# 0411tony/Yue

Hardware: AMD Instinct MI355X
Metric: BPR triplet-updates/sec at k=128 (S-round semantics, user rows sequential; the reference's exact sequential semantics: secondary.exact) (higher is better)
Workload: dtype f32

## Files before the change

### yue_amd/csrc/bpr_host.hip

```cpp
#include "host_common.hpp"

#include "train_kernels.hpp"
#include "round_kernels.hpp"

using yue_host::fail;
using yue_host::kr_of;
static_assert(yue::kNllSlots == yue_host::kNllSlotsHost && yue::kHeaderSlack == yue_host::kHeaderSlackHost, "host_common.hpp mirrors these");

namespace {

yue::TrainArgs make_args(yue_ctx *c, double lr, double regU, double regI) {
    yue::TrainArgs a{};
    a.P = c->P.p; a.Q = c->Q.p; a.dP = c->dP.p; a.dQ = c->dQ.p;
    a.stage = c->Q.p ? c->Q.p + (size_t)c->n * c->k : nullptr;
    a.ev_u = c->ev_u.p; a.ev_i = c->ev_i.p; a.ev_j = c->ev_j.p;
    a.indptr = c->indptr.p; a.indices = c->indices.p;
    a.nll_slots = c->scal.p;
    a.m = c->m; a.n = c->n; a.k = c->k;
    a.lr = lr;
    a.ru = (float)(lr * regU);
    a.ri = (float)(lr * regI);
    a.neg_lo = 0; a.neg_range = (int32_t)c->n;
    return a;
}

void launch_level(yue_ctx *c, const yue::TrainArgs &a, int64_t e0, int64_t e1) {
    const int tpw = (int)std::min<int64_t>(64, std::max<int64_t>(1, (e1 - e0) / 4096));
    const int64_t waves = (e1 - e0 + tpw - 1) / tpw;
    const dim3 grid((unsigned)((waves + 3) / 4)), block(256);
    switch (kr_of(c->k)) {
        case 1: hipLaunchKernelGGL(yue::k_bpr_level<1>, grid, block, 0, c->stream, a, e0, e1, tpw); break;
        case 2: hipLaunchKernelGGL(yue::k_bpr_level<2>, grid, block, 0, c->stream, a, e0, e1, tpw); break;
        default: hipLaunchKernelGGL(yue::k_bpr_level<4>, grid, block, 0, c->stream, a, e0, e1, tpw); break;
    }
}

int tpw_of(const yue_ctx *c, bool meta) {
    if (c->opt_round_tpw) return c->opt_round_tpw;
    const int kr = kr_of(c->k);
    return kr == 4 ? 4 : kr == 2 ? 8 : meta ? 8 : 16;
}

constexpr int64_t kMetaRangeMax = 37 * 1024;
constexpr int64_t kMetaRangesMax = 12;
constexpr int64_t kRoundGenerationsMax = 6;
constexpr double kRoundEventsPerItemRow = 4.0;
// ... 174 lines not shown
            default: return fail(YUE_ERR_ARG, "item matrices of 2 GiB and more: only the default events-per-wave setting (round_tpw = 0)");
        }
    } else
#define YUE_RM(KR_, TPW_) hipLaunchKernelGGL((yue::k_round_m<KR_, TPW_>), grid, block, 0, c->stream, a, ra, a.ev_u, a.ev_i, a.ev_j, mi, mj); break;
    switch (kr_of(c->k) * 16 + tpw) {
        case 1 * 16 + 8: YUE_RM(1, 8)
        case 1 * 16 + 16: YUE_RM(1, 16)
        case 2 * 16 + 8: YUE_RM(2, 8)
        case 4 * 16 + 4: YUE_RM(4, 4)
        case 1 * 16 + 4: YUE_RM(1, 4)
        case 2 * 16 + 4: YUE_RM(2, 4)
        case 1 * 16 + 2: YUE_RM(1, 2)
        case 2 * 16 + 2: YUE_RM(2, 2)
        default: return fail(YUE_ERR_ARG, "unsupported (k, TPW) combination");
    }
#undef YUE_RM
    launch_round_fold(c, a, e0, e1, round_index);
    return YUE_OK;
}

int launch_round_u(yue_ctx *c, const yue::TrainArgs &a, int64_t u0, int64_t u1, int64_t e0, int64_t e1, int64_t round_index) {
    yue::RoundUArgs ra{};
    ra.u_begin = u0; ra.u_end = u1; ra.ev_ptr = c->d_ev_ptr.p; ra.e_begin = e0; ra.e_end = e1; ra.staged = c->staged ? 1 : 0; ra.margins = c->margins.p;
    ra.psq_slots = c->psq_in_rounds ? c->psq_slots.p : nullptr;
    const int64_t blocks = (u1 - u0 + 3) / 4;
    if (blocks == 0) return YUE_OK;
    const dim3 grid((unsigned)blocks), block(256);
    const uint32_t *mi = c->meta_i.p, *mj = c->meta_j.p;
#define YUE_RU(KR_) do { if (c->opt_round_fast) hipLaunchKernelGGL((yue::k_round_u<KR_, true>), grid, block, 0, c->stream, a, ra, a.ev_i, a.ev_j, mi, mj); \
                         else hipLaunchKernelGGL((yue::k_round_u<KR_, false>), grid, block, 0, c->stream, a, ra, a.ev_i, a.ev_j, mi, mj); } while (0)
    switch (kr_of(c->k)) {
        case 1: YUE_RU(1); break;
        case 2: YUE_RU(2); break;
        default: YUE_RU(4); break;
    }
#undef YUE_RU
    launch_round_fold(c, a, e0, e1, round_index);
    return YUE_OK;
}

template <typename F>
int run_rounds(yue_ctx *c, yue::TrainArgs a, const std::vector<int64_t> &bounds, int apply_p, F after_round, bool meta = false, const std::vector<int64_t> *user_blocks = nullptr) {
    const int64_t R = (int64_t)bounds.size() - 1;
    int64_t widest = 0;
    for (int64_t r = 0; r < R; ++r) widest = std::max(widest, bounds[(size_t)r + 1] - bounds[(size_t)r]);
    if (widest >= (1ll << 24)) meta = false;
    const bool fits31 = (c->n + 2 * widest) * (int64_t)c->k * 4 < (1ll << 31);
// ... 57 lines not shown
        c->ev_triplets[c->ev_used] = bounds.back() - bounds.front();
        c->ev_launches[c->ev_used] = (int64_t)ne.size();
        c->ev_used++;
    }
    return YUE_OK;
}

void reset_round_state(yue_ctx *c) {
    (void)hipStreamSynchronize(c->stream);
    if (c->cnt0.p) (void)hipMemsetAsync(c->cnt0.p, 0, c->cnt0.n * sizeof(unsigned long long), c->stream);
    if (c->cnt1.p) (void)hipMemsetAsync(c->cnt1.p, 0, c->cnt1.n * sizeof(unsigned long long), c->stream);
    if (c->cntp0.p) (void)hipMemsetAsync(c->cntp0.p, 0, c->cntp0.n * sizeof(uint32_t), c->stream);
    if (c->cntp1.p) (void)hipMemsetAsync(c->cntp1.p, 0, c->cntp1.n * sizeof(uint32_t), c->stream);
    if (c->dP.p) (void)hipMemsetAsync(c->dP.p, 0, c->dP.n * sizeof(float), c->stream);
    if (c->dQ.p) (void)hipMemsetAsync(c->dQ.p, 0, c->dQ.n * sizeof(float), c->stream);
    (void)hipStreamSynchronize(c->stream);
}


}

namespace yue_host {
int zero_scalars(yue_ctx *c) {
    HIPCHK(hipMemsetAsync(c->scal.p, 0, (yue::kNllSlots + 8) * sizeof(double), c->stream));
    return YUE_OK;
}

int read_scalars(yue_ctx *c, double *nll, double *sp, double *sq) {
    double *sc = c->scal.p + yue::kNllSlots;
    hipLaunchKernelGGL(yue::k_sum_slots, dim3(1), dim3(64), 0, c->stream, c->scal.p, yue::kNllSlots, sc);
    double h[3];
    HIPCHK(hipMemcpyAsync(h, sc, sizeof h, hipMemcpyDeviceToHost, c->stream));
    HIPCHK(hipStreamSynchronize(c->stream));
    if (nll) *nll = h[0];
    if (sp) *sp = h[1];
    if (sq) *sq = h[2];
    return YUE_OK;
}

int sumsq_async(yue_ctx *c, const double *p_slots) {
    double *sc = c->scal.p + yue::kNllSlots;
    HIPCHK(hipMemsetAsync(sc + 1, 0, 2 * sizeof(double), c->stream));
    if (p_slots) hipLaunchKernelGGL(yue::k_sum_slots, dim3(1), dim3(64), 0, c->stream, p_slots, yue::kNllSlots, sc + 1);
    else hipLaunchKernelGGL(yue::k_sumsq, dim3(2048), dim3(256), 0, c->stream, c->P.p, c->m * c->k, sc + 1);
    hipLaunchKernelGGL(yue::k_sumsq, dim3(2048), dim3(256), 0, c->stream, c->Q.p, c->n * c->k, sc + 2);
    return YUE_OK;
}

int upload_triplets(yue_ctx *c, const int32_t *u, const int32_t *i, const int32_t *j, int64_t T, bool validate) {
    for (int64_t t = 0; validate && t < T; ++t) {
        if (u[t] < 0 || u[t] >= c->m || i[t] < 0 || i[t] >= c->n || j[t] >= c->n)
            return fail(YUE_ERR_ARG, "triplet " + std::to_string(t) + " out of range");
    }
// ... 143 lines not shown
    a.U = c->P.p; a.V = c->Q.p; a.gU = c->dP.p; a.gV = c->dQ.p; a.k = c->k; a.u = c->xu.p; a.i = c->xi.p; a.j = c->xj.p; a.T = T;
    a.reg = (float)reg; a.loss_slots = c->scal.p;
    const dim3 grid((unsigned)(((T + 31) / 32 + 3) / 4));
    switch (kr_of(c->k)) {
        case 1: hipLaunchKernelGGL(yue::k_mb_grad<1>, grid, dim3(256), 0, c->stream, a); break;
        case 2: hipLaunchKernelGGL(yue::k_mb_grad<2>, grid, dim3(256), 0, c->stream, a); break;
        default: hipLaunchKernelGGL(yue::k_mb_grad<4>, grid, dim3(256), 0, c->stream, a); break;
    }
    const double b1 = 0.9, b2 = 0.999;
    const float lr_t = (float)(lr * std::sqrt(1.0 - std::pow(b2, (double)step)) / (1.0 - std::pow(b1, (double)step)));
    const int64_t mk = c->m * (int64_t)c->k, nk = c->n * (int64_t)c->k;
    hipLaunchKernelGGL(yue::k_adam, dim3((unsigned)std::min<int64_t>(8192, (mk + 255) / 256)), dim3(256), 0, c->stream, c->P.p, c->aU_m.p, c->aU_v.p, c->dP.p, mk, lr_t, 0.9f, 0.999f, 1e-8f);
    hipLaunchKernelGGL(yue::k_adam, dim3((unsigned)std::min<int64_t>(8192, (nk + 255) / 256)), dim3(256), 0, c->stream, c->Q.p, c->aV_m.p, c->aV_v.p, c->dQ.p, nk, lr_t, 0.9f, 0.999f, 1e-8f);
    HIPCHK(hipGetLastError());
    return read_scalars(c, loss_out, nullptr, nullptr);
}

int yue_sample_negatives(yue_ctx *c, uint64_t seed, uint32_t epoch, int32_t *j_out) {
    if (!c || !c->have_inter || !j_out) return fail(YUE_ERR_ARG, "yue_sample_negatives: no interactions uploaded");
    HIPCHK(hipSetDevice(c->device));
    yue::TrainArgs a = make_args(c, 0, 0, 0);
    a.seed = seed; a.epoch = epoch;
    if (c->E > 0) {
        hipLaunchKernelGGL(yue::k_sample, dim3((unsigned)((c->E + 255) / 256)), dim3(256), 0, c->stream, a, c->E);
        HIPCHK(hipGetLastError());
        HIPCHK(hipMemcpyAsync(j_out, c->ev_j.p, c->E * sizeof(int32_t), hipMemcpyDeviceToHost, c->stream));
    }
    HIPCHK(hipStreamSynchronize(c->stream));
    return YUE_OK;
}

int yue_sumsq(yue_ctx *c, double *sp, double *sq) {
    if (!c || !c->have_factors) return fail(YUE_ERR_ARG, "yue_sumsq: no factors uploaded");
    HIPCHK(hipSetDevice(c->device));
    int rc = sumsq_async(c);
    if (rc) return rc;
    double h[2];
    HIPCHK(hipMemcpyAsync(h, c->scal.p + yue::kNllSlots + 1, sizeof h, hipMemcpyDeviceToHost, c->stream));
    HIPCHK(hipStreamSynchronize(c->stream));
    if (sp) *sp = h[0];
    if (sq) *sq = h[1];
    return YUE_OK;
}

int yue_bpr_epoch(yue_ctx *c, uint64_t seed, uint32_t epoch, int64_t round_events, double lr, double regU, double regI,
                  double *nll_out, double *sumsqP_out, double *sumsqQ_out) {
    if (!c || !c->have_factors || !c->have_inter) return fail(YUE_ERR_ARG, "yue_bpr_epoch: upload factors and interactions first");
    if (round_events < 0) return fail(YUE_ERR_ARG, "yue_bpr_epoch: round_events must be positive (or 0 for the device's default)");
    HIPCHK(hipSetDevice(c->device));
    yue::TrainArgs a = make_args(c, lr, regU, regI);
    a.seed = seed + 0x632BE59BD9B4E019ull * (uint64_t)c->rank;
    a.epoch = epoch;
    int rc = zero_scalars(c);
    if (rc) return rc;
    const int64_t E = c->E;
    if (E > 0) hipLaunchKernelGGL(yue::k_sample, dim3((unsigned)((E + 255) / 256)), dim3(256), 0, c->stream, a, E);
    if (c->opt_epoch_exact) {
        if (yue_host::on_communicator(c) && c->nranks > 1) return fail(YUE_ERR_ARG, "yue_bpr_epoch: option epoch_exact runs on one GPU (the sequential order spans all item shards)");
        if ((rc = yue_host::chain_epoch(c, lr, regU, regI))) return rc;
        if ((rc = sumsq_async(c))) return rc;
        return read_scalars(c, nll_out, sumsqP_out, sumsqQ_out);
    }
    std::vector<int64_t> bounds;
    double tot[2] = {(double)E, (double)c->n};
    if (yue_host::on_communicator(c)) {
        if ((rc = yue_allreduce_f64(c, tot, 2))) return rc;
        if ((rc = zero_scalars(c))) return rc;
    }
    const double etot = tot[0];
    if (round_events == 0 && (rc = default_round_events(c, tot[1] / c->nranks, &round_events))) return rc;
    int64_t ub = 1, group = 1;
    if ((rc = yue_epoch_plan(c->m, c->k, round_events, etot, c->nranks, &ub, &group, nullptr))) return rc;
    if (!yue_host::on_communicator(c)) group = std::max<int64_t>(1, (c->m + ub - 1) / ub);
    else group = std::max<int64_t>(1, ((int64_t)c->opt_comm_group_mb << 20) / std::max<int64_t>(1, ub * c->k * 4));
    std::vector<int64_t> ublock;
    for (int64_t u0 = 0; u0 < c->m; u0 += ub) { ublock.push_back(u0); bounds.push_back(c->h_ev_ptr[(size_t)u0]); }
    ublock.push_back(c->m); bounds.push_back(E);
    const int64_t R = (int64_t)ublock.size() - 1;
    const bool seq_user = !yue_host::on_communicator(c) && c->opt_round_user_seq && meta_path_fits(c);
    if (seq_user) {
        HIPCHK(c->d_ev_ptr.resize((size_t)c->m + 1));
        if (!c->d_ev_ptr_valid) {
            HIPCHK(hipMemcpyAsync(c->d_ev_ptr.p, c->h_ev_ptr.data(), ((size_t)c->m + 1) * sizeof(int64_t), hipMemcpyHostToDevice, c->stream));
            c->d_ev_ptr_valid = true;
        }
        HIPCHK(c->margins.resize((size_t)std::max<int64_t>(E, 1)));
    }
    c->psq_in_rounds = seq_user && c->all_users_have_events && E > 0;
    if (c->psq_in_rounds) {
        HIPCHK(c->psq_slots.resize((size_t)yue::kNllSlots));
        HIPCHK(hipMemsetAsync(c->psq_slots.p, 0, (size_t)yue::kNllSlots * sizeof(double), c->stream));
    }
    c->last_round_user_seq = 0;
    auto after = [&](int64_t r) -> int {
        if (seq_user && !c->bigq) { c->last_round_user_seq = 1; return YUE_OK; }
        if ((r + 1) % group != 0 && r + 1 != R) return YUE_OK;
        const int64_t g_first = ublock[(size_t)(r - (r % group))], g_last = ublock[(size_t)r + 1];
        const int64_t first = g_first * c->k, count = (g_last - g_first) * c->k;
        const dim3 grid((unsigned)std::min<int64_t>(4096, (count + 255) / 256));
        if (!yue_host::on_communicator(c)) {
            hipLaunchKernelGGL(yue::k_apply_range, grid, dim3(256), 0, c->stream, c->P.p, c->dP.p, first, count);
            return YUE_OK;
        }
        HIPCHK(hipEventRecord(c->ev_rounds, c->stream));
        HIPCHK(hipStreamWaitEvent(c->comm_stream, c->ev_rounds, 0));
        c->comm_collectives += 1;
        c->comm_bytes += (double)count * sizeof(float);
        if (const int rcr = yue_host::reduce_user_block(c, first, count, c->comm_stream)) return rcr;
        hipLaunchKernelGGL(yue::k_apply_range, grid, dim3(256), 0, c->comm_stream, c->P.p, c->dP.p, first, count);
        return YUE_OK;
    };
    c->comm_collectives = 0; c->comm_bytes = 0.0; c->comm_wait_ms = 0.0;
    if ((rc = run_rounds(c, a, bounds, 0, after, meta_path_fits(c), seq_user ? &ublock : nullptr))) { reset_round_state(c); return rc; }
    if (c->last_round_user_seq && E > 0)
        hipLaunchKernelGGL(yue::k_loss_margins, dim3(2048), dim3(256), 0, c->stream, c->margins.p, c->ev_j.p, E, c->scal.p);
    const bool psq_done = c->psq_in_rounds && c->last_round_user_seq;
    c->psq_in_rounds = false;
    if (yue_host::on_communicator(c)) {
        HIPCHK(hipEventRecord(c->ev_t_rounds, c->stream));
        HIPCHK(hipEventRecord(c->ev_t_comm, c->comm_stream));
    }
    HIPCHK(hipEventRecord(c->ev_comm, c->comm_stream));
    HIPCHK(hipStreamWaitEvent(c->stream, c->ev_comm, 0));
    c->comm_compute_waits = 1;
    HIPCHK(hipGetLastError());
    if ((rc = sumsq_async(c, psq_done ? c->psq_slots.p : nullptr))) return rc;
    if ((rc = read_scalars(c, nll_out, sumsqP_out, sumsqQ_out))) return rc;
    if (yue_host::on_communicator(c)) {
        float ms = 0.f;
        HIPCHK(hipEventSynchronize(c->ev_t_comm));
        HIPCHK(hipEventElapsedTime(&ms, c->ev_t_rounds, c->ev_t_comm));
        c->comm_wait_ms = ms > 0.f ? ms : 0.0;
    }
    return YUE_OK;
}

int yue_epoch_plan(int64_t m, int k, int64_t round_events, double events_total, int nranks,
                   int64_t *user_block, int64_t *blocks_per_group, int64_t *n_blocks) {
    if (m <= 0 || k <= 0 || round_events <= 0 || nranks < 1 || !(events_total >= 0.0)) return fail(YUE_ERR_ARG, "yue_epoch_plan: bad argument");
    const double per_user = events_total / (double)nranks / (double)m;
    const int64_t ub = std::max<int64_t>(1, (int64_t)std::floor((double)round_events / std::max(per_user, 1e-9) + 0.5));
    if (user_block) *user_block = ub;
    if (blocks_per_group) *blocks_per_group = std::max<int64_t>(1, (8ll << 20) / std::max<int64_t>(1, ub * k * 4));
    if (n_blocks) *n_blocks = (m + ub - 1) / ub;
    return YUE_OK;
}

int yue_default_round_events(yue_ctx *c, int64_t *out) {
    if (!c || !c->have_factors || !out) return fail(YUE_ERR_ARG, "yue_default_round_events: upload factors first (the value depends on k)");
    HIPCHK(hipSetDevice(c->device));
// ... 56 lines not shown
    else if (key == "scan_batch") *value = c->opt_scan_batch;
    else if (key == "scan_two_phase") *value = c->opt_scan_two_phase;
    else if (key == "fism_lds") *value = c->opt_fism_lds;
    else if (key == "fism_inplace") *value = c->opt_fism_inplace;
    else if (key == "scan_growth") *value = c->opt_scan_growth;
    else if (key == "scan_filter_ub") *value = c->opt_scan_filter_ub;
    else if (key == "scan_streams") *value = c->opt_scan_streams;
    else if (key == "scan_slabs") *value = c->opt_scan_slabs;
    else if (key == "scan_streams_min_users") *value = c->opt_scan_streams_min_users;
    else if (key == "scan_last_chunks") *value = c->scan_chunks;
    else if (key == "scan_last_few_users") *value = c->scan_few_users;
    else if (key == "scan_last_settle") *value = c->scan_settle;
    else if (key == "topn_true") *value = c->opt_topn_true;
    else if (key == "round_stage") *value = c->opt_round_stage;
    else if (key == "round_last_stage_max") *value = c->last_stage_max;
    else if (key == "round_meta") *value = c->opt_round_meta;
    else if (key == "comm_group_mb") *value = c->opt_comm_group_mb;
    else if (key == "round_cus_reserved") *value = c->opt_round_cus_reserved;
    else if (key == "comm_last_compute_waits") *value = c->comm_compute_waits;
    else if (key == "round_user_seq") *value = c->opt_round_user_seq;
    else if (key == "round_fast") *value = c->opt_round_fast;
    else if (key == "round_last_user_seq") *value = c->last_round_user_seq;
    else if (key == "round_bucket") *value = c->opt_round_bucket;
    else if (key == "fold_blocks") *value = c->opt_fold_blocks;
    else if (key == "round_tpw") *value = c->opt_round_tpw;
    else if (key == "epoch_exact") *value = c->opt_epoch_exact;
    else if (key == "replay_levels") *value = c->opt_replay_levels;
    else if (key == "chain_waves") *value = c->opt_chain_waves;
    else if (key == "chain_split") *value = c->opt_chain_split;
    else if (key == "chain_fast") *value = c->opt_chain_fast;
    else if (key == "chain_xcd") *value = c->opt_chain_xcd;
    else if (key == "chain_last_us") *value = c->chain_kernel_us;
    else if (key == "chain_ring") *value = c->opt_chain_ring;
    else if (key == "chain_spin") *value = c->opt_chain_spin;
    else if (key == "chain_last_runs") *value = c->chain_runs;
    else if (key == "chain_last_waves") *value = c->chain_waves;
    else if (key == "replay_last_levels") *value = c->replay_levels;
    else if (key == "round_path") *value = fold_path(c) ? 1 : 0;
    else if (key.compare(0, 5, "wrmf_") == 0) return yue_host::wrmf_get_option(c, key, value);
    else if (key.compare(0, 4, "knn_") == 0) return yue_host::knn_get_option(c, key, value);
    else if (key.compare(0, 4, "ipf_") == 0) return yue_host::ipf_get_option(c, key, value);
    else return fail(YUE_ERR_ARG, "yue_get_option: unknown option " + key);
    return YUE_OK;
}

int yue_set_option(yue_ctx *c, const char *name, int64_t value) {
// ... 25 lines not shown
        hipStream_t fresh = nullptr;
        if (value == 0) HIPCHK(hipStreamCreateWithFlags(&fresh, hipStreamNonBlocking));
        else {
            std::vector<uint32_t> mask((size_t)(cus + 31) / 32, 0u);
            for (int cu = 0; cu < cus - (int)value; ++cu) mask[(size_t)cu / 32] |= 1u << (cu % 32);
            HIPCHK(hipExtStreamCreateWithCUMask(&fresh, (uint32_t)mask.size(), mask.data()));
        }
        (void)hipStreamDestroy(c->stream);
        c->stream = fresh;
        c->opt_round_cus_reserved = (int)value;
        return YUE_OK;
    }
    if (key == "round_user_seq") { c->opt_round_user_seq = value != 0; return YUE_OK; }
    if (key == "round_fast") { c->opt_round_fast = value != 0; return YUE_OK; }
    if (key == "epoch_exact") { c->opt_epoch_exact = value != 0; return YUE_OK; }
    if (key == "replay_levels") { c->opt_replay_levels = value != 0; return YUE_OK; }
    if (key == "chain_split") { if (value < -1 || value > 1) return fail(YUE_ERR_ARG, "yue_set_option: chain_split must be -1, 0 or 1"); c->opt_chain_split = (int)value; return YUE_OK; }
    if (key == "chain_fast") { c->opt_chain_fast = value != 0; return YUE_OK; }
    if (key == "chain_xcd") { c->opt_chain_xcd = value != 0; return YUE_OK; }
    if (key == "chain_ring") { if (value != 0 && value != 8 && value != 16) return fail(YUE_ERR_ARG, "yue_set_option: chain_ring must be 0, 8 or 16"); c->opt_chain_ring = (int)value; return YUE_OK; }
    if (key == "chain_waves") { if (value < 0 || value > 8) return fail(YUE_ERR_ARG, "yue_set_option: chain_waves must be 0..8"); c->opt_chain_waves = (int)value; return YUE_OK; }
    if (key == "chain_spin") { if (value < 0 || value > 0x7fffffff) return fail(YUE_ERR_ARG, "yue_set_option: chain_spin out of range"); c->opt_chain_spin = value; return YUE_OK; }
    if (key == "round_bucket") { c->opt_round_bucket = value != 0; return YUE_OK; }
    if (key == "fold_blocks") { if (value < 1 || value > 65536) return fail(YUE_ERR_ARG, "yue_set_option: fold_blocks out of range"); c->opt_fold_blocks = (int)value; return YUE_OK; }
#ifdef YUE_STAMPS
    if (key == "debug_stamp_launch") { c->stamp_launch = value; c->update_launches = 0; return YUE_OK; }
#endif
    if (key == "round_tpw") {
        if (value != 0 && value != 2 && value != 4 && value != 8 && value != 16) return fail(YUE_ERR_ARG, "yue_set_option: round_tpw must be 0, 2, 4, 8 or 16");
        if (value == 8 && kr_of(c->k) == 4) return fail(YUE_ERR_ARG, "yue_set_option: round_tpw 8 needs k <= 128");
        if (value == 16 && kr_of(c->k) != 1) return fail(YUE_ERR_ARG, "yue_set_option: round_tpw 16 needs k <= 64");
        c->opt_round_tpw = (int)value;
        return YUE_OK;
    }
    if (key.compare(0, 5, "wrmf_") == 0) return yue_host::wrmf_set_option(c, key, value);
    if (key.compare(0, 4, "knn_") == 0) return yue_host::knn_set_option(c, key, value);
    if (key.compare(0, 4, "ipf_") == 0) return yue_host::ipf_set_option(c, key, value);
    return fail(YUE_ERR_ARG, "yue_set_option: unknown option " + key);
}

#ifdef YUE_STAMPS
int yue_debug_get_stamps(yue_ctx *c, unsigned long long *out, int64_t max_waves, int64_t *n_waves) {
    HIPCHK(hipStreamSynchronize(c->stream));
    const int64_t w = std::min(max_waves, c->stamp_waves);
    if (w > 0) HIPCHK(hipMemcpy(out, c->stamps.p, (size_t)w * 64, hipMemcpyDeviceToHost));
    *n_waves = w;
// ... 6 lines not shown
```

### yue_amd/csrc/core_host.hip

```cpp
#include "host_common.hpp"

namespace yue_host {
thread_local std::string g_err;
int fail(int code, const std::string &msg) { g_err = msg; return code; }
}
using yue_host::fail;
void yue_comm_release(yue_ctx *c);

extern "C" {

const char *yue_last_error(void) { return yue_host::g_err.c_str(); }
int yue_version(void) { return 1; }

int yue_ctx_create(int device, yue_ctx **out) {
    if (!out) return fail(YUE_ERR_ARG, "yue_ctx_create: out is NULL");
    int ndev = 0;
    HIPCHK(hipGetDeviceCount(&ndev));
    if (ndev <= 0) return fail(YUE_ERR_HIP, "no HIP device visible: libyue_hip needs an MI355X (no CPU fallback exists)");
    if (device < 0 || device >= ndev) return fail(YUE_ERR_ARG, "device ordinal out of range");
    HIPCHK(hipSetDevice(device));
    yue_ctx *c = new yue_ctx();
    c->device = device;
    const auto init = [c]() -> int {
        HIPCHK(hipStreamCreateWithFlags(&c->stream, hipStreamNonBlocking));
        HIPCHK(hipStreamCreateWithFlags(&c->comm_stream, hipStreamNonBlocking));
        HIPCHK(hipEventCreateWithFlags(&c->ev_rounds, hipEventDisableTiming));
        HIPCHK(hipEventCreateWithFlags(&c->ev_comm, hipEventDisableTiming));
        HIPCHK(hipEventCreate(&c->ev_t_rounds));
        HIPCHK(hipEventCreate(&c->ev_t_comm));
        HIPCHK(hipEventCreate(&c->ev_scan0));
        HIPCHK(hipEventCreate(&c->ev_scan1));
        HIPCHK(c->scal.resize(yue_host::kNllSlotsHost + 8));
        return YUE_OK;
    };
    const int rc = init();
    if (rc) { const std::string msg = yue_host::g_err; (void)yue_ctx_destroy(c); yue_host::g_err = msg; return rc; }
    *out = c;
    return YUE_OK;
}

int yue_ctx_destroy(yue_ctx *c) {
    if (!c) return YUE_OK;
    (void)hipSetDevice(c->device);
    if (c->stream) (void)hipStreamSynchronize(c->stream);
    if (c->comm_stream) (void)hipStreamSynchronize(c->comm_stream);
    yue_comm_release(c);
    if (c->comm_stream) (void)hipStreamDestroy(c->comm_stream);
    if (c->ev_rounds) (void)hipEventDestroy(c->ev_rounds);
    if (c->ev_comm) (void)hipEventDestroy(c->ev_comm);
    if (c->ev_t_rounds) (void)hipEventDestroy(c->ev_t_rounds);
    if (c->ev_t_comm) (void)hipEventDestroy(c->ev_t_comm);
    if (c->ev_scan0) (void)hipEventDestroy(c->ev_scan0);
    if (c->ev_chain0) (void)hipEventDestroy(c->ev_chain0);
    if (c->ev_chain1) (void)hipEventDestroy(c->ev_chain1);
    if (c->ev_scan1) (void)hipEventDestroy(c->ev_scan1);
// ... 110 lines not shown
```

### yue_amd/csrc/host_common.hpp

```cpp
#pragma once
#include "../../include/yue_hip.h"

#include <hip/hip_runtime.h>

#include <algorithm>
#include <cmath>
#include <cstdio>
#include <cstdlib>
#include <cstring>
#include <string>
#include <vector>

struct ncclComm;
struct yue_wrmf;
struct yue_knn;
struct yue_ipf;

namespace yue_host {

int fail(int code, const std::string &msg);

#define HIPCHK(expr)                                                                              \
    do {                                                                                          \
        hipError_t e_ = (expr);                                                                   \
        if (e_ != hipSuccess)                                                                     \
            return yue_host::fail(YUE_ERR_HIP, std::string(#expr) + ": " + hipGetErrorString(e_)); \
    } while (0)

template <typename T>
struct DevBuf {
    T *p = nullptr;
    size_t n = 0;
    hipError_t resize(size_t count) {
        if (count <= n && p) return hipSuccess;
        if (p) { hipError_t e = hipFree(p); p = nullptr; n = 0; if (e != hipSuccess) return e; }
        if (count == 0) return hipSuccess;
        hipError_t e = hipMalloc((void **)&p, count * sizeof(T));
        if (e == hipSuccess) n = count;
        return e;
    }
    void release() { if (p) (void)hipFree(p); p = nullptr; n = 0; }
};

constexpr int kNllSlotsHost = 1024;
constexpr int kHeaderSlackHost = 16;

inline int kr_of(int k) { return k <= 64 ? 1 : k <= 128 ? 2 : 4; }

}

using yue_host::DevBuf;

struct yue_ctx {
    int device = 0;
    hipStream_t stream = nullptr;
    int64_t m = 0, n = 0, E = 0, nnz = 0;
    int k = 0;
    bool have_factors = false, have_inter = false;
    DevBuf<float> P, Q, dP, dQ;
    DevBuf<float> margins;
    DevBuf<double> psq_slots;
    DevBuf<unsigned long long> cnt0, cnt1;
    DevBuf<uint32_t> cntp0, cntp1;
    DevBuf<uint32_t> tab0, tab1;
    bool staged = false;
    bool bigq = false;
    DevBuf<uint32_t> meta_i, meta_j;
    DevBuf<unsigned long long> round_rows;
    DevBuf<uint2> fold, bk_touch;
    DevBuf<uint32_t> bk_ptr;
    DevBuf<int64_t> d_bounds;
    std::vector<int64_t> h_bounds;
#ifdef YUE_STAMPS
    DevBuf<unsigned long long> stamps;
    int64_t stamp_launch = -1, update_launches = 0, stamp_waves = 0;
#endif
    DevBuf<int32_t> ev_u, ev_i, ev_j, indices;
    DevBuf<int64_t> indptr;
    DevBuf<int32_t> xu, xi, xj, xk;
    DevBuf<double> x_loss;
    DevBuf<float> aU_m, aU_v, aV_m, aV_v;
    int64_t adam_m = 0, adam_n = 0; int adam_k = 0;
    DevBuf<double> scal;
    std::vector<int64_t> h_ev_ptr;
// ... 6 lines not shown
    DevBuf<int64_t> s_mask_ptr;
    DevBuf<float> s_scores, s_row, s_norms;
    double scan_ms = 0.0;
    int64_t scan_events = 0, scan_rescored = 0, scan_tiles_done = 0, scan_tiles_total = 0;
    DevBuf<unsigned long long> s_work;
    DevBuf<unsigned short> s_qb;
    DevBuf<uint32_t> s_masks;
    int opt_scan_two_phase = 1;
    int64_t opt_scan_streams_min_users = 262144;
    int opt_scan_slabs = 4;
    int opt_scan_streams = 2;
    int opt_scan_filter_ub = 3;
    int opt_scan_growth = 0;
    int scan_chunks = 0;
    int scan_used_bf16 = 0;
    int opt_scan_f32 = 0;
    int opt_scan_batch = 0;
    int opt_round_tpw = 0;
    int opt_topn_true = 0;
    int scan_settle = 0;
    int last_stage_max = 0;
    int opt_round_stage = 1;
    int opt_round_bucket = 0;
    int opt_fold_blocks = 1536;
    int opt_round_user_seq = 1;
    int opt_round_fast = 1;
    int last_round_user_seq = 0;
    int opt_comm_group_mb = 8;
    int opt_round_cus_reserved = 0;
    int64_t comm_compute_waits = 0;
    int opt_round_meta = 1;
    int timing_stride = 0;
    std::vector<std::pair<hipEvent_t, hipEvent_t>> ev_pool;
    std::vector<int64_t> ev_triplets, ev_launches;
    size_t ev_used = 0;
    DevBuf<double> fP, fBi, f_coef, f_x, f_hist, f_scores, f_out_sc;
    DevBuf<float> fQ;
    DevBuf<int64_t> f_ptr;
    DevBuf<int32_t> f_items, f_negs, f_ids, f_flags;
    DevBuf<int64_t> f_uq_ptr, f_neg_ptr;
    DevBuf<int32_t> f_uq_items, f_loc_i, f_loc_j;
    DevBuf<float> f_wq, f_dQ;
    DevBuf<double> f_wp, f_wb, f_dP, f_dB;
    DevBuf<unsigned> f_cnt;
    int64_t fn = 0;
    int fk = 0;
// ... 17 lines not shown
    int64_t opt_chain_spin = 0;
    int64_t chain_runs = 0, chain_waves = 0, chain_groups = 0, chain_kernel_us = 0, replay_levels = 0;
    hipEvent_t ev_chain0 = nullptr, ev_chain1 = nullptr;
    ncclComm *comm = nullptr;
    int rank = 0, nranks = 1;
    hipStream_t comm_stream = nullptr;
    hipEvent_t ev_rounds = nullptr, ev_comm = nullptr;
    hipEvent_t ev_t_rounds = nullptr, ev_t_comm = nullptr;
    int (*seam_reduce)(void *host, int64_t count, int dtype, void *user) = nullptr;
    void *seam_user = nullptr;
    std::vector<float> seam_buf;
    int64_t comm_collectives = 0;
    double comm_bytes = 0.0, comm_wait_ms = 0.0;
    int comm_version = 0, comm_nranks_reported = 0;
    hipEvent_t ev_scan0 = nullptr, ev_scan1 = nullptr;
    yue_wrmf *wrmf = nullptr;
    yue_knn *knn = nullptr;
    yue_ipf *ipf = nullptr;
};

namespace yue_host {
inline bool on_communicator(const yue_ctx *c) { return c->comm != nullptr || c->seam_reduce != nullptr; }
int zero_scalars(yue_ctx *c);
int read_scalars(yue_ctx *c, double *nll, double *sp, double *sq);
int sumsq_async(yue_ctx *c, const double *p_slots = nullptr);
int upload_triplets(yue_ctx *c, const int32_t *u, const int32_t *i, const int32_t *j, int64_t T, bool validate);
int reduce_user_block(yue_ctx *c, int64_t first, int64_t count, hipStream_t stream);
int chain_epoch(yue_ctx *c, double lr, double regU, double regI);
int chain_stream(yue_ctx *c, int64_t T, double lr, double regU, double regI);
void wrmf_release(yue_ctx *c);
int wrmf_set_option(yue_ctx *c, const std::string &key, int64_t value);
int wrmf_get_option(yue_ctx *c, const std::string &key, int64_t *value);
void knn_release(yue_ctx *c);
int knn_set_option(yue_ctx *c, const std::string &key, int64_t value);
int knn_get_option(yue_ctx *c, const std::string &key, int64_t *value);
void ipf_release(yue_ctx *c);
int ipf_set_option(yue_ctx *c, const std::string &key, int64_t value);
int ipf_get_option(yue_ctx *c, const std::string &key, int64_t *value);
}
```

### yue_amd/csrc/round_kernels.hpp

```cpp
#pragma once
#include "train_kernels.hpp"

#ifdef YUE_ABL_NO_HOT
#define YUE_M_HOT(val, rs, vo, so) asm volatile("" :: "v"(val))
#else
#define YUE_M_HOT(val, rs, vo, so) YUE_BATOMIC(val, rs, vo, so)
#endif
#ifdef YUE_ABL_NO_DP
#define YUE_M_DP(val, rs, vo, so) asm volatile("" :: "v"(val))
#else
#define YUE_M_DP(val, rs, vo, so) YUE_BATOMIC(val, rs, vo, so)
#endif

#define YUE_BLOAD_NT(rs, vo, so) __builtin_bit_cast(float, __builtin_amdgcn_raw_buffer_load_b32((rs), (vo), (so), 2))
#if defined(YUE_EXP_LOAD_CACHED)
#define YUE_M_LOAD_J(rs, vo, so) YUE_BLOAD(rs, vo, so)
#define YUE_M_LOAD_I(rs, vo, so) YUE_BLOAD(rs, vo, so)
#elif defined(YUE_EXP_LOAD_NT)
#define YUE_M_LOAD_J(rs, vo, so) YUE_BLOAD_NT(rs, vo, so)
#define YUE_M_LOAD_I(rs, vo, so) YUE_BLOAD_NT(rs, vo, so)
#else
#define YUE_M_LOAD_J(rs, vo, so) YUE_BLOAD_NT(rs, vo, so)
#define YUE_M_LOAD_I(rs, vo, so) YUE_BLOAD(rs, vo, so)
#endif

#define YUE_FOLD_LD(p) __builtin_nontemporal_load(p)
#define YUE_FOLD_LDROW(p) (*(p))

namespace yue {

constexpr uint32_t kMetaStageMax = 64u;
constexpr uint32_t kMetaStageDefault = 4u;
constexpr uint32_t kMetaUnique = 1u, kMetaStaged = 2u, kMetaHot = 3u;
constexpr uint32_t kMetaFirst = 1u << 31;
constexpr int kMetaUnroll = 8;
__host__ __device__ inline uint32_t meta_kind(uint32_t w) { return w & 3u; }
__host__ __device__ inline uint32_t meta_slot(uint32_t w) { return (w >> 2) & 0x1fffffffu; }
__host__ __device__ inline bool meta_first(uint32_t w) { return (w & kMetaFirst) != 0u; }
__host__ __device__ inline uint32_t fold_count(uint32_t w) { return w >> 25; }
__host__ __device__ inline uint32_t fold_block(uint32_t w) { return w & 0x1ffffffu; }
constexpr uint32_t kLdsStaged = 1u << 31, kLdsTicket = 1u << 25;
static_assert(kMetaStageMax <= 64u, "tickets of a block must fit bits 25..30 of the LDS word");
__device__ inline uint32_t meta_of_staged(uint32_t lds) {
    const uint32_t ticket = (lds >> 25) & 63u;
    return kMetaStaged | (((lds & 0x1ffffffu) + ticket) << 2) | (ticket == 0u ? kMetaFirst : 0u);
}

struct MetaArgs {
    const int32_t *ev_i, *ev_j;
// ... 437 lines not shown
            } else {
#pragma unroll
                for (int r = 0; r < KR; ++r) YUE_M_HOT(o[r].qi2 - qi[r], rsdQ, vo[r], oi);
            }
            if (clj != kMetaHot) {
#pragma unroll
                for (int r = 0; r < KR; ++r) YUE_BSTORE(full_j ? o[r].qj2 : o[r].qj2 - qj[r], rsQ, vo[r], wj);
            } else {
#pragma unroll
                for (int r = 0; r < KR; ++r) YUE_M_HOT(o[r].qj2 - qj[r], rsdQ, vo[r], oj);
            }
        };
        constexpr int D = KR == 1 ? 8 : 4;
        float qi[D][KR], qj[D][KR];
#pragma unroll
        for (int s_ = 0; s_ < D; ++s_) gather(qi[s_], qj[s_], (unsigned)s_);
        for (unsigned t = 0; t < seg_len; t += D) {
#pragma unroll
            for (int s_ = 0; s_ < D; ++s_) {
                step(qi[s_], qj[s_], t + s_);
                gather(qi[s_], qj[s_], (t + s_ + D) & 63u);
            }
        }
        if ((unsigned)lane < seg_len) ra.margins[e0 + seg + lane] = xs;
    }
#pragma unroll
    for (int r = 0; r < KR; ++r) { const unsigned e = 64u * r + lane; if (e < k) prow[e] = p[r]; }
    if (ra.psq_slots) {
        double s = 0.0;
#pragma unroll
        for (int r = 0; r < KR; ++r) { const unsigned e = 64u * r + lane; const float sq = p[r] * p[r]; if (e < k) s += (double)sq; }
#pragma unroll
        for (int off = 1; off < 64; off <<= 1) s += __shfl_xor(s, off);
        if (lane == 0) atomicAdd(ra.psq_slots + (u & (kNllSlots - 1)), s);
    }
}

__global__ void __launch_bounds__(256) k_loss_margins(const float *__restrict__ x, const int32_t *__restrict__ evj, int64_t E, double *nll_slots) {
    double nl = 0.0;
    const int64_t stride = (int64_t)gridDim.x * blockDim.x;
    for (int64_t e = (int64_t)blockIdx.x * blockDim.x + threadIdx.x; e < E; e += stride)
        if (evj[e] >= 0) nl += -log(chain_sigmoid(x[e]));
#pragma unroll
    for (int off = 1; off < 64; off <<= 1) nl += __shfl_xor(nl, off);
    if ((threadIdx.x & 63) == 0 && nl != 0.0) atomicAdd(nll_slots + ((blockIdx.x * 4 + (threadIdx.x >> 6)) & (kNllSlots - 1)), nl);
}

struct FoldArgs {
    const uint2 *fold;
    const unsigned long long *round_rows;
    float *Q, *dQ;
    const float *stage;
    int k;
    uint32_t capacity;
};

template <int KR, int EPG>
__device__ __forceinline__ void fold_group(const FoldArgs &f, int lane, unsigned k, uint32_t nact, const uint2 (&ent)[4]) {
    float st[EPG][4][KR];
    unsigned el[KR];
    bool big = false;
#pragma unroll
    for (int r = 0; r < KR; ++r) el[r] = min(64u * r + lane, k - 1u);
#pragma unroll
    for (int sl = 0; sl < EPG; ++sl) {
        if ((uint32_t)sl >= nact) continue;
        const uint32_t c = fold_count(ent[sl].y);
        const bool hot = c == 0u;
// ... 102 lines not shown
```

### yue_amd/csrc/train_kernels.hpp

```cpp
#pragma once
#include "bpr_device.hpp"

namespace yue {

__global__ void __launch_bounds__(256) k_sample(TrainArgs a, int64_t E) {
    int64_t e = (int64_t)blockIdx.x * blockDim.x + threadIdx.x;
    if (e < E) a.ev_j[e] = sample_negative(a, a.ev_u[e], e);
}

template <int KR>
__global__ void __launch_bounds__(256) k_bpr_level(TrainArgs a, int64_t e_begin, int64_t e_end, int tpw) {
    const int lane = threadIdx.x & 63;
    const int64_t wave = (int64_t)blockIdx.x * (blockDim.x >> 6) + (threadIdx.x >> 6);
    const int64_t base = e_begin + wave * tpw;
    if (base >= e_end) return;
    const int cnt = (int)((e_end - base) < (int64_t)tpw ? (e_end - base) : (int64_t)tpw);
    int u = 0, i = 0, j = 0;
    if (lane < cnt) { u = a.ev_u[base + lane]; i = a.ev_i[base + lane]; j = a.ev_j[base + lane]; }
    const int k = a.k;
    double nll = 0.0;
    for (int t = 0; t < cnt; ++t) {
        const int64_t tu = __builtin_amdgcn_readlane(u, t);
        const int64_t ti = __builtin_amdgcn_readlane(i, t);
        const int64_t tj = __builtin_amdgcn_readlane(j, t);
        float p[KR], qi[KR], qj[KR];
#pragma unroll
        for (int r = 0; r < KR; ++r) {
            const int e = 64 * r + lane;
            p[r] = e < k ? a.P[tu * k + e] : 0.0f;
            qi[r] = e < k ? a.Q[ti * k + e] : 0.0f;
// ... 482 lines not shown
```

Measured before the change: 1.846 billion.

## Add row-cooperative negative sampling and fuse epoch loss/sumsq reductions into one kernel

Adds k_sample_rows, where each wave handles a few users and draws negatives for all of a user's events together. It checks each candidate against the user's interaction row with a shuffle-based binary search over 64-wide chunks. This path is chosen by default when there are at least 8 events per user. It also replaces the separate loss-margin, sumsq and slot-sum launches with a single k_epoch_sums kernel. Rejected triplets now store an infinite margin, so the loss pass no longer reads ev_j. The per-user P-norm slots move into the scalar buffer, which drops a separate allocation and memset. The cost is a more complex sampler whose correctness depends on sorted per-user index rows.

```diff
diff --git a/yue_amd/csrc/bpr_host.hip b/yue_amd/csrc/bpr_host.hip
--- a/yue_amd/csrc/bpr_host.hip
+++ b/yue_amd/csrc/bpr_host.hip
@@ -22,6 +22,30 @@
     a.ri = (float)(lr * regI);
     a.neg_lo = 0; a.neg_range = (int32_t)c->n;
     return a;
+}
+
+constexpr int kScalWords = yue_host::kScalWordsHost;
+static_assert(kScalWords == 2 * yue::kNllSlots + 8, "host_common.hpp mirrors the layout");
+double *psq_slots(yue_ctx *c) { return c->scal.p + yue::kNllSlots + 8; }
+
+int upload_ev_ptr(yue_ctx *c) {
+    HIPCHK(c->d_ev_ptr.resize((size_t)c->m + 1));
+    if (!c->d_ev_ptr_valid) {
+        HIPCHK(hipMemcpyAsync(c->d_ev_ptr.p, c->h_ev_ptr.data(), ((size_t)c->m + 1) * sizeof(int64_t), hipMemcpyHostToDevice, c->stream));
+        c->d_ev_ptr_valid = true;
+    }
+    return YUE_OK;
+}
+
+constexpr int64_t kSampleRowsMinEvents = 8;
+int launch_sample(yue_ctx *c, const yue::TrainArgs &a) {
+    const bool rows = c->opt_sample_form == 2 || (c->opt_sample_form == 0 && c->E >= kSampleRowsMinEvents * c->m);
+    if (rows) {
+        const int rc = upload_ev_ptr(c);
+        if (rc) return rc;
+        hipLaunchKernelGGL(yue::k_sample_rows, dim3((unsigned)((c->m + yue::kSampleUsersPerBlock - 1) / yue::kSampleUsersPerBlock)), dim3(256), 0, c->stream, a, c->d_ev_ptr.p);
+    } else hipLaunchKernelGGL(yue::k_sample, dim3((unsigned)((c->E + 255) / 256)), dim3(256), 0, c->stream, a, c->E);
+    return YUE_OK;
 }
 
 void launch_level(yue_ctx *c, const yue::TrainArgs &a, int64_t e0, int64_t e1) {
@@ -242,7 +266,7 @@
 int launch_round_u(yue_ctx *c, const yue::TrainArgs &a, int64_t u0, int64_t u1, int64_t e0, int64_t e1, int64_t round_index) {
     yue::RoundUArgs ra{};
     ra.u_begin = u0; ra.u_end = u1; ra.ev_ptr = c->d_ev_ptr.p; ra.e_begin = e0; ra.e_end = e1; ra.staged = c->staged ? 1 : 0; ra.margins = c->margins.p;
-    ra.psq_slots = c->psq_in_rounds ? c->psq_slots.p : nullptr;
+    ra.psq_slots = c->psq_in_rounds ? psq_slots(c) : nullptr;
     const int64_t blocks = (u1 - u0 + 3) / 4;
     if (blocks == 0) return YUE_OK;
     const dim3 grid((unsigned)blocks), block(256);
@@ -346,13 +370,13 @@
 
 namespace yue_host {
 int zero_scalars(yue_ctx *c) {
-    HIPCHK(hipMemsetAsync(c->scal.p, 0, (yue::kNllSlots + 8) * sizeof(double), c->stream));
-    return YUE_OK;
-}
-
-int read_scalars(yue_ctx *c, double *nll, double *sp, double *sq) {
+    HIPCHK(hipMemsetAsync(c->scal.p, 0, (size_t)kScalWords * sizeof(double), c->stream));
+    return YUE_OK;
+}
+
+int read_scalars(yue_ctx *c, double *nll, double *sp, double *sq, bool sum_slots) {
     double *sc = c->scal.p + yue::kNllSlots;
-    hipLaunchKernelGGL(yue::k_sum_slots, dim3(1), dim3(64), 0, c->stream, c->scal.p, yue::kNllSlots, sc);
+    if (sum_slots) hipLaunchKernelGGL(yue::k_sum_slots, dim3(1), dim3(64), 0, c->stream, c->scal.p, yue::kNllSlots, sc);
     double h[3];
     HIPCHK(hipMemcpyAsync(h, sc, sizeof h, hipMemcpyDeviceToHost, c->stream));
     HIPCHK(hipStreamSynchronize(c->stream));
@@ -542,7 +566,8 @@
     yue::TrainArgs a = make_args(c, 0, 0, 0);
     a.seed = seed; a.epoch = epoch;
     if (c->E > 0) {
-        hipLaunchKernelGGL(yue::k_sample, dim3((unsigned)((c->E + 255) / 256)), dim3(256), 0, c->stream, a, c->E);
+        const int rc = launch_sample(c, a);
+        if (rc) return rc;
         HIPCHK(hipGetLastError());
         HIPCHK(hipMemcpyAsync(j_out, c->ev_j.p, c->E * sizeof(int32_t), hipMemcpyDeviceToHost, c->stream));
     }
@@ -574,7 +599,7 @@
     int rc = zero_scalars(c);
     if (rc) return rc;
     const int64_t E = c->E;
-    if (E > 0) hipLaunchKernelGGL(yue::k_sample, dim3((unsigned)((E + 255) / 256)), dim3(256), 0, c->stream, a, E);
+    if (E > 0 && (rc = launch_sample(c, a))) return rc;
     if (c->opt_epoch_exact) {
         if (yue_host::on_communicator(c) && c->nranks > 1) return fail(YUE_ERR_ARG, "yue_bpr_epoch: option epoch_exact runs on one GPU (the sequential order spans all item shards)");
         if ((rc = yue_host::chain_epoch(c, lr, regU, regI))) return rc;
@@ -599,18 +624,10 @@
     const int64_t R = (int64_t)ublock.size() - 1;
     const bool seq_user = !yue_host::on_communicator(c) && c->opt_round_user_seq && meta_path_fits(c);
     if (seq_user) {
-        HIPCHK(c->d_ev_ptr.resize((size_t)c->m + 1));
-        if (!c->d_ev_ptr_valid) {
-            HIPCHK(hipMemcpyAsync(c->d_ev_ptr.p, c->h_ev_ptr.data(), ((size_t)c->m + 1) * sizeof(int64_t), hipMemcpyHostToDevice, c->stream));
-            c->d_ev_ptr_valid = true;
-        }
+        if ((rc = upload_ev_ptr(c))) return rc;
         HIPCHK(c->margins.resize((size_t)std::max<int64_t>(E, 1)));
     }
     c->psq_in_rounds = seq_user && c->all_users_have_events && E > 0;
-    if (c->psq_in_rounds) {
-        HIPCHK(c->psq_slots.resize((size_t)yue::kNllSlots));
-        HIPCHK(hipMemsetAsync(c->psq_slots.p, 0, (size_t)yue::kNllSlots * sizeof(double), c->stream));
-    }
     c->last_round_user_seq = 0;
     auto after = [&](int64_t r) -> int {
         if (seq_user && !c->bigq) { c->last_round_user_seq = 1; return YUE_OK; }
@@ -632,8 +649,7 @@
     };
     c->comm_collectives = 0; c->comm_bytes = 0.0; c->comm_wait_ms = 0.0;
     if ((rc = run_rounds(c, a, bounds, 0, after, meta_path_fits(c), seq_user ? &ublock : nullptr))) { reset_round_state(c); return rc; }
-    if (c->last_round_user_seq && E > 0)
-        hipLaunchKernelGGL(yue::k_loss_margins, dim3(2048), dim3(256), 0, c->stream, c->margins.p, c->ev_j.p, E, c->scal.p);
+    const bool sums_fused = c->last_round_user_seq && E > 0;
     const bool psq_done = c->psq_in_rounds && c->last_round_user_seq;
     c->psq_in_rounds = false;
     if (yue_host::on_communicator(c)) {
@@ -644,8 +660,12 @@
     HIPCHK(hipStreamWaitEvent(c->stream, c->ev_comm, 0));
     c->comm_compute_waits = 1;
     HIPCHK(hipGetLastError());
-    if ((rc = sumsq_async(c, psq_done ? c->psq_slots.p : nullptr))) return rc;
-    if ((rc = read_scalars(c, nll_out, sumsqP_out, sumsqQ_out))) return rc;
+    if (sums_fused) {
+        hipLaunchKernelGGL(yue::k_epoch_sums, dim3(2048), dim3(256), 0, c->stream, c->margins.p, E, psq_done ? psq_slots(c) : nullptr,
+                           c->P.p, c->m * (int64_t)c->k, c->Q.p, c->n * (int64_t)c->k, c->scal.p + yue::kNllSlots);
+        HIPCHK(hipGetLastError());
+    } else if ((rc = sumsq_async(c, psq_done ? psq_slots(c) : nullptr))) return rc;
+    if ((rc = read_scalars(c, nll_out, sumsqP_out, sumsqQ_out, !sums_fused))) return rc;
     if (yue_host::on_communicator(c)) {
         float ms = 0.f;
         HIPCHK(hipEventSynchronize(c->ev_t_comm));
@@ -748,6 +768,7 @@
     else if (key == "round_fast") *value = c->opt_round_fast;
     else if (key == "round_last_user_seq") *value = c->last_round_user_seq;
     else if (key == "round_bucket") *value = c->opt_round_bucket;
+    else if (key == "sample_form") *value = c->opt_sample_form;
     else if (key == "fold_blocks") *value = c->opt_fold_blocks;
     else if (key == "round_tpw") *value = c->opt_round_tpw;
     else if (key == "epoch_exact") *value = c->opt_epoch_exact;
@@ -819,6 +840,7 @@
     if (key == "chain_waves") { if (value < 0 || value > 8) return fail(YUE_ERR_ARG, "yue_set_option: chain_waves must be 0..8"); c->opt_chain_waves = (int)value; return YUE_OK; }
     if (key == "chain_spin") { if (value < 0 || value > 0x7fffffff) return fail(YUE_ERR_ARG, "yue_set_option: chain_spin out of range"); c->opt_chain_spin = value; return YUE_OK; }
     if (key == "round_bucket") { c->opt_round_bucket = value != 0; return YUE_OK; }
+    if (key == "sample_form") { if (value < 0 || value > 2) return fail(YUE_ERR_ARG, "yue_set_option: sample_form must be 0, 1 or 2"); c->opt_sample_form = (int)value; return YUE_OK; }
     if (key == "fold_blocks") { if (value < 1 || value > 65536) return fail(YUE_ERR_ARG, "yue_set_option: fold_blocks out of range"); c->opt_fold_blocks = (int)value; return YUE_OK; }
 #ifdef YUE_STAMPS
     if (key == "debug_stamp_launch") { c->stamp_launch = value; c->update_launches = 0; return YUE_OK; }
diff --git a/yue_amd/csrc/core_host.hip b/yue_amd/csrc/core_host.hip
--- a/yue_amd/csrc/core_host.hip
+++ b/yue_amd/csrc/core_host.hip
@@ -30,7 +30,7 @@
         HIPCHK(hipEventCreate(&c->ev_t_comm));
         HIPCHK(hipEventCreate(&c->ev_scan0));
         HIPCHK(hipEventCreate(&c->ev_scan1));
-        HIPCHK(c->scal.resize(yue_host::kNllSlotsHost + 8));
+        HIPCHK(c->scal.resize(yue_host::kScalWordsHost));
         return YUE_OK;
     };
     const int rc = init();
diff --git a/yue_amd/csrc/host_common.hpp b/yue_amd/csrc/host_common.hpp
--- a/yue_amd/csrc/host_common.hpp
+++ b/yue_amd/csrc/host_common.hpp
@@ -44,6 +44,7 @@
 
 constexpr int kNllSlotsHost = 1024;
 constexpr int kHeaderSlackHost = 16;
+constexpr int kScalWordsHost = 2 * kNllSlotsHost + 8;
 
 inline int kr_of(int k) { return k <= 64 ? 1 : k <= 128 ? 2 : 4; }
 
@@ -59,7 +60,6 @@
     bool have_factors = false, have_inter = false;
     DevBuf<float> P, Q, dP, dQ;
     DevBuf<float> margins;
-    DevBuf<double> psq_slots;
     DevBuf<unsigned long long> cnt0, cnt1;
     DevBuf<uint32_t> cntp0, cntp1;
     DevBuf<uint32_t> tab0, tab1;
@@ -112,6 +112,7 @@
     int last_stage_max = 0;
     int opt_round_stage = 1;
     int opt_round_bucket = 0;
+    int opt_sample_form = 0;
     int opt_fold_blocks = 1536;
     int opt_round_user_seq = 1;
     int opt_round_fast = 1;
@@ -175,7 +176,7 @@
 namespace yue_host {
 inline bool on_communicator(const yue_ctx *c) { return c->comm != nullptr || c->seam_reduce != nullptr; }
 int zero_scalars(yue_ctx *c);
-int read_scalars(yue_ctx *c, double *nll, double *sp, double *sq);
+int read_scalars(yue_ctx *c, double *nll, double *sp, double *sq, bool sum_slots = true);
 int sumsq_async(yue_ctx *c, const double *p_slots = nullptr);
 int upload_triplets(yue_ctx *c, const int32_t *u, const int32_t *i, const int32_t *j, int64_t T, bool validate);
 int reduce_user_block(yue_ctx *c, int64_t first, int64_t count, hipStream_t stream);
diff --git a/yue_amd/csrc/round_kernels.hpp b/yue_amd/csrc/round_kernels.hpp
--- a/yue_amd/csrc/round_kernels.hpp
+++ b/yue_amd/csrc/round_kernels.hpp
@@ -24,7 +24,11 @@
 #define YUE_M_LOAD_I(rs, vo, so) YUE_BLOAD(rs, vo, so)
 #endif
 
+#if defined(YUE_EXP_FOLD_CACHED)
+#define YUE_FOLD_LD(p) (*(p))
+#else
 #define YUE_FOLD_LD(p) __builtin_nontemporal_load(p)
+#endif
 #define YUE_FOLD_LDROW(p) (*(p))
 
 namespace yue {
@@ -508,7 +512,7 @@
                 gather(qi[s_], qj[s_], (t + s_ + D) & 63u);
             }
         }
-        if ((unsigned)lane < seg_len) ra.margins[e0 + seg + lane] = xs;
+        if ((unsigned)lane < seg_len) ra.margins[e0 + seg + lane] = hJ < 0 ? __builtin_inff() : xs;
     }
 #pragma unroll
     for (int r = 0; r < KR; ++r) { const unsigned e = 64u * r + lane; if (e < k) prow[e] = p[r]; }
@@ -522,14 +526,29 @@
     }
 }
 
-__global__ void __launch_bounds__(256) k_loss_margins(const float *__restrict__ x, const int32_t *__restrict__ evj, int64_t E, double *nll_slots) {
-    double nl = 0.0;
-    const int64_t stride = (int64_t)gridDim.x * blockDim.x;
-    for (int64_t e = (int64_t)blockIdx.x * blockDim.x + threadIdx.x; e < E; e += stride)
-        if (evj[e] >= 0) nl += -log(chain_sigmoid(x[e]));
-#pragma unroll
-    for (int off = 1; off < 64; off <<= 1) nl += __shfl_xor(nl, off);
-    if ((threadIdx.x & 63) == 0 && nl != 0.0) atomicAdd(nll_slots + ((blockIdx.x * 4 + (threadIdx.x >> 6)) & (kNllSlots - 1)), nl);
+__global__ void __launch_bounds__(256) k_epoch_sums(const float *__restrict__ x, int64_t E, const double *__restrict__ p_slots,
+                                                    const float *__restrict__ P, int64_t np, const float *__restrict__ Q, int64_t nq, double *out) {
+    __shared__ double part[3][4];
+    double s[3] = {0.0, 0.0, 0.0};
+    const int64_t stride = (int64_t)gridDim.x * blockDim.x, t0 = (int64_t)blockIdx.x * blockDim.x + threadIdx.x;
+    for (int64_t e = t0; e < E; e += stride) s[0] += -log(chain_sigmoid(x[e]));
+    if (p_slots) {
+        if (blockIdx.x == 0) for (int t = threadIdx.x; t < kNllSlots; t += 256) s[1] += p_slots[t];
+    } else {
+        for (int64_t t = t0; t < np; t += stride) { const float sq = P[t] * P[t]; s[1] += (double)sq; }
+    }
+    for (int64_t t = t0; t < nq; t += stride) { const float sq = Q[t] * Q[t]; s[2] += (double)sq; }
+#pragma unroll
+    for (int q = 0; q < 3; ++q) {
+#pragma unroll
+        for (int off = 1; off < 64; off <<= 1) s[q] += __shfl_xor(s[q], off);
+        if ((threadIdx.x & 63) == 0) part[q][threadIdx.x >> 6] = s[q];
+    }
+    __syncthreads();
+    if (threadIdx.x < 3) {
+        const double v = part[threadIdx.x][0] + part[threadIdx.x][1] + part[threadIdx.x][2] + part[threadIdx.x][3];
+        if (v != 0.0) atomicAdd(out + threadIdx.x, v);
+    }
 }
 
 struct FoldArgs {
diff --git a/yue_amd/csrc/train_kernels.hpp b/yue_amd/csrc/train_kernels.hpp
--- a/yue_amd/csrc/train_kernels.hpp
+++ b/yue_amd/csrc/train_kernels.hpp
@@ -6,6 +6,46 @@
 __global__ void __launch_bounds__(256) k_sample(TrainArgs a, int64_t E) {
     int64_t e = (int64_t)blockIdx.x * blockDim.x + threadIdx.x;
     if (e < E) a.ev_j[e] = sample_negative(a, a.ev_u[e], e);
+}
+
+__device__ __forceinline__ bool row64_contains(int32_t row, int32_t x) {
+    int pos = 0;
+#pragma unroll
+    for (int step = 32; step >= 1; step >>= 1) pos += __shfl(row, pos + step - 1) < x ? step : 0;
+    return __shfl(row, pos) == x;
+}
+
+constexpr int kSampleUsers = 4, kSampleUsersPerBlock = 4 * kSampleUsers;
+__global__ void __launch_bounds__(256) k_sample_rows(TrainArgs a, const int64_t *__restrict__ ev_ptr) {
+    const int lane = threadIdx.x & 63;
+    const int64_t u0 = ((int64_t)blockIdx.x * 4 + (threadIdx.x >> 6)) * kSampleUsers;
+    if (u0 >= a.m) return;
+    const int64_t uq = u0 + lane < a.m ? u0 + lane : a.m;
+    const int64_t evp = lane <= kSampleUsers ? ev_ptr[uq] : 0, rwp = lane <= kSampleUsers ? a.indptr[uq] : 0;
+    int64_t e0[kSampleUsers], e1[kSampleUsers], r0[kSampleUsers], len[kSampleUsers];
+    int32_t first[kSampleUsers];
+#pragma unroll
+    for (int q = 0; q < kSampleUsers; ++q) {
+        e0[q] = __shfl(evp, q); e1[q] = __shfl(evp, q + 1);
+        r0[q] = __shfl(rwp, q); len[q] = __shfl(rwp, q + 1) - r0[q];
+        first[q] = lane < len[q] && e1[q] > e0[q] ? a.indices[r0[q] + lane] : INT32_MAX;
+    }
+#pragma unroll
+    for (int q = 0; q < kSampleUsers; ++q) {
+        for (int64_t eb = e0[q]; eb < e1[q]; eb += 64) {
+            const int64_t e = eb + lane;
+            int32_t j = -1;
+            bool open = e < e1[q];
+            for (uint32_t t = 0; t < (uint32_t)kMaxAttempts && __ballot(open) != 0ull; ++t) {
+                const int32_t c = ctr_draw(a.seed, a.epoch, (uint64_t)e, t, a.neg_lo, a.neg_range);
+                bool hit = row64_contains(first[q], c);
+                for (int64_t rb = 64; rb < len[q]; rb += 64)
+                    hit = row64_contains(rb + lane < len[q] ? a.indices[r0[q] + rb + lane] : INT32_MAX, c) || hit;
+                if (open && !hit) { j = c; open = false; }
+            }
+            if (e < e1[q]) a.ev_j[e] = j;
+        }
+    }
 }
 
 template <int KR>
```

New measurement: 1.874 billion (median of 6 runs). 1.5% higher.
